# daxiongpro/EPNet

Measured on AMD Instinct MI355X. Metric: SA-stack points/sec per GPU (16384-pt KITTI scene) + % HBM roofline, higher is better.
Workload: dtype f32; 1 GPU; 256 x 16384-pt kitti scenes per GPU per step through the 4-level SA op stack (4 samplings [FPS + centre gather; levels 2-4 nested in level 1 where tie-free] + 8 ball_query + 8 fused groupings [xyz - centre ; features]), pyramid 16384>4096>1024>256>64, radii [[.1,.5],[.5,1],[1,2],[2,4]], nsample [16,32], C=0/96/256/512, HIP-graph launch; levels=4, scenes_per_gpu=256, software_pipelined=True, pipeline_stages=2, parallelism=scene-parallel x1

## Files before the change

epnet_amd/csrc/fps.hip:

```cpp
#include <math.h>

#include <type_traits>

#include "common.h"
#include "dpp.h"
#include "spatial.h"

extern "C" __device__ int epnet_llvm_writelane_i32(int, int, int) __asm("llvm.amdgcn.writelane.i32");

namespace epnet {

__device__ __forceinline__ int writelane_i32(int value, int lane, int old) {
    return epnet_llvm_writelane_i32(value, lane, old);
}

__device__ __forceinline__ unsigned bitrev_lg(unsigned v, int lg) {
    return lg == 0 ? 0u : (__brev(v) >> (32 - lg));
}

__device__ __forceinline__ int wave_max_i32(int v) {
    const int r = row16_max(v);
    const int a = __builtin_amdgcn_readlane(r, 0), b = __builtin_amdgcn_readlane(r, 16);
    const int c = __builtin_amdgcn_readlane(r, 32), d = __builtin_amdgcn_readlane(r, 48);
    return max(max(a, b), max(c, d));
}

constexpr int kIdxBuf = 4096;

__device__ __forceinline__ int fps_point_of(int q, int slot, int R, int J, int lg_bs) {
    const int r = q * R + slot / J;
    return (int)bitrev_lg((unsigned)r, lg_bs) + (slot % J) * (1 << lg_bs);
}

template <int PPT>
__device__ __forceinline__ void find_slot(const int (&t)[PPT], const float (&x)[PPT], const float (&y)[PPT],
                                          const float (&z)[PPT], const int (&g)[(PPT + 3) / 4], int wl, int target,
                                          int &slot, float &sx, float &sy, float &sz) {
    slot = 0;
    sx = sy = sz = 0.f;
    if constexpr (PPT >= 8) {
        constexpr int NG = PPT / 4;
        int grp = 0;
#pragma unroll
        for (int gi = NG - 1; gi >= 0; --gi)
            if (__builtin_amdgcn_readlane(g[gi], wl) == target) grp = gi;
#pragma unroll
        for (int gi = 0; gi < NG; ++gi)
            if (grp == gi) {
#pragma unroll
                for (int j = 4 * gi + 3; j >= 4 * gi; --j)
                    if (__builtin_amdgcn_readlane(t[j], wl) == target) slot = j;
            }
#pragma unroll
        for (int j = 0; j < PPT; ++j)
            if (slot == j) {
                sx = __int_as_float(__builtin_amdgcn_readlane(__float_as_int(x[j]), wl));
                sy = __int_as_float(__builtin_amdgcn_readlane(__float_as_int(y[j]), wl));
                sz = __int_as_float(__builtin_amdgcn_readlane(__float_as_int(z[j]), wl));
            }
    } else {
#pragma unroll
        for (int j = PPT - 1; j >= 0; --j)
            if (__builtin_amdgcn_readlane(t[j], wl) == target) {
                slot = j;
                sx = __int_as_float(__builtin_amdgcn_readlane(__float_as_int(x[j]), wl));
                sy = __int_as_float(__builtin_amdgcn_readlane(__float_as_int(y[j]), wl));
                sz = __int_as_float(__builtin_amdgcn_readlane(__float_as_int(z[j]), wl));
            }
    }
}

__device__ __forceinline__ bool fps_prologue(int m, const int *__restrict__ skip, int *__restrict__ idx_scene,
                                             int *__restrict__ prefix_out, int init) {
    const int have = skip ? skip[blockIdx.x] : 0;
    if (init >= 0) {
        if (threadIdx.x == 0 && prefix_out) prefix_out[blockIdx.x] = have >= m ? have : init;
        for (int i = threadIdx.x; i < min(have, m); i += blockDim.x) idx_scene[i] = i;
    }
    return have >= m;
}

template <int W, int PPT>
__global__ __launch_bounds__(64 * W) void fps_wave_kernel(int n, int m, int lg_bs, const float *__restrict__ xyz,
                                                          float *__restrict__ temp, int *__restrict__ idxs,
                                                          const int *__restrict__ skip, int *__restrict__ prefix_out = nullptr,
                                                          int prologue_init = -1) {
    if (fps_prologue(m, skip, idxs + (size_t)blockIdx.x * m, prefix_out, prologue_init)) return;
    __shared__ int s_val[2][16];
    __shared__ float4 s_rec[2][16];
    __shared__ int s_idx[kIdxBuf];
    constexpr int T = 64 * W;
    const int q = threadIdx.x;
    const int lane = q & 63, wave = q >> 6;
    const int bs = 1 << lg_bs;
    const int R = bs / T, J = (n + bs - 1) / bs;
    const int used = R * J;
    xyz += (size_t)blockIdx.x * n * 3;
    if (temp) temp += (size_t)blockIdx.x * n;
    idxs += (size_t)blockIdx.x * m;
    const int kNeg1 = __float_as_int(-1.f);

    float x[PPT], y[PPT], z[PPT];
    int t[PPT];
#pragma unroll
    for (int s = 0; s < PPT; ++s) {
        const int k = s < used ? fps_point_of(q, s, R, J, lg_bs) : n;
        if (k < n) {
            x[s] = xyz[k * 3 + 0];
            y[s] = xyz[k * 3 + 1];
            z[s] = xyz[k * 3 + 2];
            t[s] = __float_as_int(temp ? temp[k] : 1e10f);
        } else {
            x[s] = y[s] = z[s] = 0.f;
            t[s] = kNeg1;
        }
    }
    if (W > 1 && q < 32) s_val[q >> 4][q & 15] = kNeg1;
    if (q == 0) s_idx[0] = 0;
    float x1 = xyz[0], y1 = xyz[1], z1 = xyz[2];
    __syncthreads();

    for (int it = 1; it < m; ++it) {
        int g[(PPT + 3) / 4];
        int best = kNeg1;
        if constexpr (PPT >= 8) {
#pragma unroll
            for (int gi = 0; gi < PPT / 4; ++gi) {
                int gm = kNeg1;
#pragma unroll
                for (int j = 4 * gi; j < 4 * gi + 4; ++j) {
                    const float dx = x[j] - x1, dy = y[j] - y1, dz = z[j] - z1;
                    const float d = dx * dx + dy * dy + dz * dz;
                    t[j] = min(__float_as_int(d), t[j]);
                    gm = max(gm, t[j]);
                }
                g[gi] = gm;
                best = max(best, gm);
            }
        } else {
#pragma unroll
            for (int j = 0; j < PPT; ++j) {
                const float dx = x[j] - x1, dy = y[j] - y1, dz = z[j] - z1;
                const float d = dx * dx + dy * dy + dz * dz;
                t[j] = min(__float_as_int(d), t[j]);
                best = max(best, t[j]);
            }
            g[0] = best;
        }
        const int wbest = wave_max_i32(best);
        const unsigned long long tied = __ballot(best == wbest);
        const int wl = (int)__builtin_ctzll(tied);
        int slot;
        float sx, sy, sz;
        find_slot<PPT>(t, x, y, z, g, wl, wbest, slot, sx, sy, sz);
        const int code = ((wave * 64 + wl) << 8) | slot;
        if constexpr (W == 1) {
            x1 = sx;
            y1 = sy;
            z1 = sz;
            s_idx[it & (kIdxBuf - 1)] = code;
        } else {
            const int buf = it & 1;
            if (lane == 0) {
                s_val[buf][wave] = wbest;
                s_rec[buf][wave] = make_float4(sx, sy, sz, __int_as_float(code));
            }
            __syncthreads();
            const int wv = s_val[buf][lane & 15];
            const float4 rec = s_rec[buf][lane & 15];
            const int bm = row16_max(wv);
            const unsigned long long wtied = __ballot(wv == bm) & 0xFFFFull;
            const int ww = (int)__builtin_ctzll(wtied);
            x1 = __int_as_float(__builtin_amdgcn_readlane(__float_as_int(rec.x), ww));
            y1 = __int_as_float(__builtin_amdgcn_readlane(__float_as_int(rec.y), ww));
            z1 = __int_as_float(__builtin_amdgcn_readlane(__float_as_int(rec.z), ww));
            const int wcode = __builtin_amdgcn_readlane(__float_as_int(rec.w), ww);
            if (wave == 0) s_idx[it & (kIdxBuf - 1)] = wcode;
        }
        if ((it & (kIdxBuf - 1)) == kIdxBuf - 1 && wave == 0) {
            const int base = it - (kIdxBuf - 1);
            for (int e = lane; e < kIdxBuf; e += 64) {
                const int c = s_idx[e];
                idxs[base + e] = fps_point_of(c >> 8, c & 0xFF, R, J, lg_bs);
            }
        }
    }
    if (wave == 0) {
        const int base = (m - 1) & ~(kIdxBuf - 1);
        for (int e = lane; base + e < m; e += 64) {
            const int c = s_idx[e];
            idxs[base + e] = fps_point_of(c >> 8, c & 0xFF, R, J, lg_bs);
        }
    }
    if (temp) {
#pragma unroll
        for (int s = 0; s < PPT; ++s) {
            const int k = s < used ? fps_point_of(q, s, R, J, lg_bs) : n;
            if (k < n) temp[k] = __int_as_float(t[s]);
        }
    }
}

namespace pruned {

#ifndef EPNET_FPS_PRIO
#define EPNET_FPS_PRIO 3
#endif

#ifdef EPNET_FPS_STATS
__device__ unsigned long long g_stats[16];
#define EPNET_STAMP(var) const unsigned long long var = __builtin_amdgcn_s_memtime()
#define EPNET_ACC(slot, a, b) st_acc[slot] += (unsigned long long)((b) - (a))
#define EPNET_CNT(slot, v) st_acc[slot] += (unsigned long long)(v)
#define EPNET_STATS_BEGIN unsigned long long st_acc[8] = {0, 0, 0, 0, 0, 0, 0, 0}
#define EPNET_STATS_END if ((threadIdx.x & 63) == 0) for (int s_ = 0; s_ < 8; ++s_) atomicAdd(&g_stats[s_], st_acc[s_])
#else
#define EPNET_STAMP(var)
#define EPNET_ACC(slot, a, b)
#define EPNET_CNT(slot, v)
#define EPNET_STATS_BEGIN
#define EPNET_STATS_END
#endif

__device__ __forceinline__ unsigned rank14(int k) { return (bitrev_lg((unsigned)k & 1023u, 10) << 4) | ((unsigned)k >> 10); }
__device__ __forceinline__ int unrank14(unsigned r) { return (int)(bitrev_lg(r >> 4, 10) + ((r & 15u) << 10)); }

template <int G>
__device__ __forceinline__ int group_max(int v) {
    v = max(v, dpp_i32<0xB1>(v));
    v = max(v, dpp_i32<0x4E>(v));
    v = max(v, dpp_i32<0x141>(v));
    if (G >= 16) v = max(v, dpp_i32<0x140>(v));
    if (G >= 32) {
        const auto a = __builtin_amdgcn_permlane16_swap((unsigned)v, (unsigned)v, false, false);
        v = max((int)a[0], (int)a[1]);
    }
    return v;
}
template <int G>
__device__ __forceinline__ float group_minf(float v) {
    v = fminf(v, __int_as_float(dpp_i32<0xB1>(__float_as_int(v))));
    v = fminf(v, __int_as_float(dpp_i32<0x4E>(__float_as_int(v))));
    v = fminf(v, __int_as_float(dpp_i32<0x141>(__float_as_int(v))));
    if (G >= 16) v = fminf(v, __int_as_float(dpp_i32<0x140>(__float_as_int(v))));
    if (G >= 32) {
        const auto a = __builtin_amdgcn_permlane16_swap(__float_as_uint(v), __float_as_uint(v), false, false);
        v = fminf(__uint_as_float(a[0]), __uint_as_float(a[1]));
    }
    return v;
}
template <int G>
__device__ __forceinline__ float group_maxf(float v) { return -group_minf<G>(-v); }

template <int P>
__device__ __forceinline__ int period_max(int v) {
    if (P > 1) v = max(v, dpp_i32<0xB1>(v));
    if (P > 2) v = max(v, dpp_i32<0x4E>(v));
    if (P > 4) v = max(v, dpp_i32<0x124>(v));
    if (P > 8) v = max(v, dpp_i32<0x128>(v));
    return v;
}
template <int P>
__device__ __forceinline__ unsigned period_min(unsigned v) {
    if (P > 1) v = min(v, dpp_u32<0xB1>(v));
    if (P > 2) v = min(v, dpp_u32<0x4E>(v));
    if (P > 4) v = min(v, dpp_u32<0x124>(v));
    if (P > 8) v = min(v, dpp_u32<0x128>(v));
    return v;
}

template <int PPT>
__device__ __forceinline__ unsigned fold_parts(unsigned long long a) {
    if (PPT <= 32) a |= a >> 32;
    if (PPT <= 16) a |= a >> 16;
    if (PPT <= 8) a |= a >> 8;
    return (unsigned)a & (PPT >= 32 ? 0xFFFFFFFFu : ((1u << PPT) - 1u));
}

constexpr int kIdxBufP = 1024;

template <typename VH>
__device__ __forceinline__ unsigned rank_of(const VH &rk2, int j) {
    return ((unsigned)rk2[j >> 1] >> ((j & 1) << 4)) & 0xFFFFu;
}
template <typename VH>
__device__ __forceinline__ void set_rank(VH &rk2, int j, unsigned r) {
    rk2[j >> 1] = (j & 1) ? (int)(((unsigned)rk2[j >> 1] & 0xFFFFu) | (r << 16)) : (int)r;
}

template <int kW, int PPT, typename VF, typename VI, typename VH>
__device__ __forceinline__ void fps_rounds(int m, const VF &x, const VF &y, const VF &z, VI &t, const VH &rk2,
                                           float cx, float cy, float cz, int *__restrict__ idxs,
                                           int *__restrict__ tie_free = nullptr, int known = 0,
                                           const float *__restrict__ xyz_in_order = nullptr, int detect_upto = 0x7fffffff) {
    __shared__ unsigned long long s_key[3];
    __shared__ float4 s_rec[2][64 * kW];
    __shared__ int s_idx[kIdxBufP];
    const int q = threadIdx.x;
    const int lane = q & 63, wave = q >> 6;
    const int sub = lane & (PPT - 1);
    const int kNeg1 = __float_as_int(-1.f);

    int bm = kNeg1;
    float lox = 0.f, hix = 0.f, loy = 0.f, hiy = 0.f, loz = 0.f, hiz = 0.f;
    for (int j = 0; j < PPT; ++j) {
        const float xj = x[j], yj = y[j], zj = z[j];
        const int tj = t[j];
        const bool real = tj != kNeg1;
        const float mnx = group_minf<PPT>(real ? xj : 3.4e38f), mxx = group_maxf<PPT>(real ? xj : -3.4e38f);
        const float mny = group_minf<PPT>(real ? yj : 3.4e38f), mxy = group_maxf<PPT>(real ? yj : -3.4e38f);
        const float mnz = group_minf<PPT>(real ? zj : 3.4e38f), mxz = group_maxf<PPT>(real ? zj : -3.4e38f);
        const int gm = group_max<PPT>(tj);
        if (sub == j) {
            const bool any = gm != kNeg1;
            bm = gm;
            lox = any ? mnx : 0.f; hix = any ? mxx : 0.f;
            loy = any ? mny : 0.f; hiy = any ? mxy : 0.f;
            loz = any ? mnz : 0.f; hiz = any ? mxz : 0.f;
        }
    }
    if (q < 3) s_key[q] = 0ull;
    if (q == 0) s_idx[0] = 0;
    if (known > kIdxBufP || known > m || !xyz_in_order) known = 0;
    for (int i = q; i < known; i += 64 * kW) s_idx[i] = (int)rank14(i);
    __syncthreads();
    for (int it = 1; it < known; ++it) {
        const float px = __builtin_amdgcn_fmed3f(cx, lox, hix), py = __builtin_amdgcn_fmed3f(cy, loy, hiy),
                    pz = __builtin_amdgcn_fmed3f(cz, loz, hiz);
        const float bdx = px - cx, bdy = py - cy, bdz = pz - cz;
        const float L = bdx * bdx + bdy * bdy + bdz * bdz;
        unsigned active = fold_parts<PPT>(__ballot(__float_as_int(L) < bm));
        const float nx = xyz_in_order[it * 3 + 0], ny = xyz_in_order[it * 3 + 1], nz = xyz_in_order[it * 3 + 2];
        while (active) {
            const int j = (int)__builtin_ctz(active);
            active &= active - 1u;
            const float xj = x[j], yj = y[j], zj = z[j];
            const int told = t[j];
            __builtin_amdgcn_sched_barrier(0);
            const float dx = xj - cx, dy = yj - cy, dz = zj - cz;
            const float d = dx * dx + dy * dy + dz * dz;
            const int tj = min(__float_as_int(d), told);
            t[j] = tj;
            const int gm = group_max<PPT>(tj);
            bm = (sub == j) ? gm : bm;
// ... 388 lines not shown
                const int e1 = two ? s_ * 64 + (int)__builtin_ctzll(act) : e0;
                act &= act - 1ull;
                const Row r0 = load_row(e0);
                Row r1 = r0;
                if (two) r1 = load_row(e1);
                finish(e0, r0, true, cx, cy, cz);
                if (two) finish(e1, r1, true, cx, cy, cz);
            }
        }
        if (stale) {
            stale = false;
            int lmax = bm[0];
#pragma unroll
            for (int s_ = 1; s_ < kBPL; ++s_) lmax = max(lmax, bm[s_]);
            wbest = wave_max_all(lmax);
            unsigned lrank = 0xFFFFFFFFu;
            float lx = 0.f, ly = 0.f, lz = 0.f;
#pragma unroll
            for (int s_ = 0; s_ < kBPL; ++s_) {
                const bool take = bm[s_] == wbest && bm[s_] != kNeg1 && brank[s_] < lrank;
                lrank = take ? brank[s_] : lrank;
                lx = take ? bxx[s_] : lx;
                ly = take ? byy[s_] : ly;
                lz = take ? bzz[s_] : lz;
            }
            unsigned long long cand = __ballot(lrank != 0xFFFFFFFFu);
            if (cand & (cand - 1ull)) {
                const unsigned rmin = wave_min_all(lrank);
                cand = __ballot(lrank == rmin);
            }
            publisher = cand != 0ull && lane == (int)__builtin_ctzll(cand);
            pub_rank = lrank;
            pub_x = lx; pub_y = ly; pub_z = lz;
        }
        const int buf = it & 1;
        if (publisher) {
            s_rec[buf][wave] = make_float4(pub_x, pub_y, pub_z, 0.f);
            const unsigned long long key =
                ((unsigned long long)(unsigned)wbest << 32) | (unsigned long long)(((0xFFFFu - pub_rank) << 4) | (unsigned)wave);
            __hip_atomic_fetch_max(&s_key[kb], key, __ATOMIC_RELAXED, __HIP_MEMORY_SCOPE_WORKGROUP);
        }
        __syncthreads();
        const unsigned klo = (unsigned)s_key[kb];
        const float4 rec = s_rec[buf][klo & 15u];
        cx = rec.x;
        cy = rec.y;
        cz = rec.z;
        const int kb2 = kb == 0 ? 2 : kb - 1;
        kb = kb == 2 ? 0 : kb + 1;
        if (wave == 0) {
            s_idx[it & (kIdxBufP - 1)] = (int)(0xFFFFu - (klo >> 4));
            if (lane == 0) s_key[kb2] = 0ull;
            if ((it & (kIdxBufP - 1)) == kIdxBufP - 1) {
                const int base = it - (kIdxBufP - 1);
                for (int e = lane; e < kIdxBufP; e += 64) idxs[base + e] = unrank16((unsigned)s_idx[e]);
            }
        }
    }
    if (wave == 0) {
        const int base = (m - 1) & ~(kIdxBufP - 1);
        for (int e = lane; base + e < m; e += 64) idxs[base + e] = unrank16((unsigned)s_idx[e]);
    }
    __builtin_amdgcn_s_setprio(0);
    for (int e = 0; e < nmine; ++e) {
        const int pos = (bid(e) << 6) + lane;
        if (pos < n) temp[__float_as_int(sorted[pos].w)] = tsort[pos];
    }
}

}


__device__ __forceinline__ unsigned fps_rank(int k, int lg) {
    return (bitrev_lg((unsigned)k & ((1u << lg) - 1u), lg) << 20) | ((unsigned)k >> lg);
}

__device__ __forceinline__ int fps_unrank(unsigned rank, int lg) {
    return (int)(bitrev_lg(rank >> 20, lg) + ((rank & 0xFFFFFu) << lg));
}

__device__ __forceinline__ long long wave_max_i64(long long v) {
#pragma unroll
    for (int off = 32; off >= 1; off >>= 1) {
        const long long o = __shfl_xor(v, off, 64);
        v = o > v ? o : v;
    }
    return v;
}

__global__ __launch_bounds__(1024) void fps_stream_kernel(int n, int m, int lg_bs, const float *__restrict__ xyz,
                                                          float *__restrict__ temp, int *__restrict__ idxs,
                                                          const int *__restrict__ skip) {
    if (skip && skip[blockIdx.x] >= m) return;
    __shared__ long long red[2][16];
    const int BS = blockDim.x;
    const int q = threadIdx.x;
    const int lane = q & 63, wave = q >> 6;
    xyz += (size_t)blockIdx.x * n * 3;
    temp += (size_t)blockIdx.x * n;
    idxs += (size_t)blockIdx.x * m;
    if (q < 32) red[q >> 4][q & 15] = (long long)0x8000000000000000ull;
    if (q == 0) idxs[0] = 0;
    float x1 = xyz[0], y1 = xyz[1], z1 = xyz[2];
    __syncthreads();
    for (int it = 1; it < m; ++it) {
        float best = -1.f;
        int bestk = q;
        for (int k = q; k < n; k += BS) {
            const float dx = xyz[k * 3 + 0] - x1, dy = xyz[k * 3 + 1] - y1, dz = xyz[k * 3 + 2] - z1;
            const float d = dx * dx + dy * dy + dz * dz;
            const float d2 = fminf(d, temp[k]);
            temp[k] = d2;
            bestk = d2 > best ? k : bestk;
            best = d2 > best ? d2 : best;
        }
        const unsigned rank = fps_rank(bestk, lg_bs);
        long long key = ((long long)__float_as_int(best) << 32) | (long long)(0x7FFFFFFFu - rank);
        key = wave_max_i64(key);
        if (lane == 0) red[it & 1][wave] = key;
        __syncthreads();
        long long kk = red[it & 1][lane & 15];
#pragma unroll
        for (int off = 8; off >= 1; off >>= 1) {
            const long long o = __shfl_xor(kk, off, 64);
            kk = o > kk ? o : kk;
        }
        const unsigned wr = 0x7FFFFFFFu - (unsigned)(kk & 0xFFFFFFFFll);
        const int old = __builtin_amdgcn_readfirstlane(fps_unrank(wr, lg_bs));
        x1 = xyz[old * 3 + 0];
        y1 = xyz[old * 3 + 1];
        z1 = xyz[old * 3 + 2];
        if (q == 0) idxs[it] = old;
    }
}

static int ref_block_lg(int work_size) {
    int pow_2 = (int)(std::log(static_cast<double>(work_size)) / std::log(2.0));
    if (pow_2 > 10) pow_2 = 10;
    if (pow_2 < 0) pow_2 = 0;
    return pow_2;
}

}

using namespace epnet;

__global__ void fps_prefix_kernel(int m, const int *__restrict__ skip, int *__restrict__ idx, int *__restrict__ prefix_out, int init);

static bool fps_prune_applies(int n, int m) {
    return tuning(kFpsPrune) != 0 && n > 1024 && n > tuning(kFpsPruneMin) && n <= 16384 && m > 1;
}

static int fps_plain(int b, int n, int m, const float *xyz, float *temp, int *idx, const int *skip, int *prefix_out,
                     epnet_stream_t stream, int prefix_cap = 0x7fffffff, int prologue_init = -1) {
    EPNET_REQUIRE(b >= 0 && n >= 1 && m >= 0);
    if (b == 0 || m == 0) return EPNET_OK;
    EPNET_REQUIRE(xyz && idx);
    if ((long long)n > (1ll << 20) * 1024) return EPNET_ELIMIT;
    hipStream_t s = (hipStream_t)stream;
    const int lg = ref_block_lg(n);
    const int bs_ref = 1 << lg;
    dim3 grid(b);
    const int J = div_up(n, bs_ref);
    auto prefix_first = [&]() -> int {
        if (prologue_init < 0) return EPNET_OK;
        hipLaunchKernelGGL(fps_prefix_kernel, dim3(b), dim3(256), 0, s, m, skip, idx, prefix_out, prologue_init);
        return check_launch("sampling prefix");
    };
    if (fps_prune_applies(n, m)) {
        if (int rc = prefix_first()) return rc;
        int waves = n > 8192 ? 8 : 4;
        const int w = tuning(kFpsPwaves);
        if (w > 0 && div_up(n, 64 * w) <= 32) waves = w;
        const int ppt_need = div_up(n, 64 * waves);
        const int ppt = ppt_need <= 8 ? 8 : ppt_need <= 16 ? 16 : 32;
        const size_t lds = (size_t)(kCells + kCells / (kCells / (64 * waves)) + 64) * sizeof(int) + (size_t)64 * waves * ppt * 2;
#define EPNET_FPS_PRUNED(W_, P_) \
    hipLaunchKernelGGL((pruned::fps_pruned_kernel<W_, P_>), grid, dim3(64 * W_), lds, s, n, m, xyz, temp, idx, skip, prefix_out, prefix_cap)
        if (waves == 8) {
            if (ppt == 8) EPNET_FPS_PRUNED(8, 8);
            else if (ppt == 16) EPNET_FPS_PRUNED(8, 16);
            else EPNET_FPS_PRUNED(8, 32);
        } else {
            if (ppt == 8) EPNET_FPS_PRUNED(4, 8);
            else if (ppt == 16) EPNET_FPS_PRUNED(4, 16);
            else EPNET_FPS_PRUNED(4, 32);
        }
#undef EPNET_FPS_PRUNED
        return check_launch("furthest_point_sampling");
    }
    if (bs_ref >= 64 && J <= 16) {
        int waves = bs_ref / 64;
        for (int w = 1; w <= bs_ref / 64; w *= 2)
            if ((bs_ref / (64 * w)) * J <= 16) {
                waves = w;
                break;
            }
        if (n > 512 && b <= 512 && bs_ref / 64 >= 8 && waves < 8) waves = 8;
        const int w = tuning(kFpsWaves);
        if (w >= 1 && w <= bs_ref / 64 && (bs_ref / (64 * w)) * J <= 16) waves = w;
        const int ppt = (bs_ref / (64 * waves)) * J;
#define EPNET_FPS_LAUNCH(W_, P_) \
    hipLaunchKernelGGL((fps_wave_kernel<W_, P_>), grid, dim3(64 * W_), 0, s, n, m, lg, xyz, temp, idx, skip, prefix_out, prologue_init)
#define EPNET_FPS_PPT(W_)                      \
    do {                                       \
        if (ppt <= 1) EPNET_FPS_LAUNCH(W_, 1); \
        else if (ppt <= 2) EPNET_FPS_LAUNCH(W_, 2); \
        else if (ppt <= 4) EPNET_FPS_LAUNCH(W_, 4); \
        else if (ppt <= 8) EPNET_FPS_LAUNCH(W_, 8); \
        else EPNET_FPS_LAUNCH(W_, 16);         \
    } while (0)
        switch (waves) {
            case 1: EPNET_FPS_PPT(1); break;
            case 2: EPNET_FPS_PPT(2); break;
            case 4: EPNET_FPS_PPT(4); break;
            case 8: EPNET_FPS_PPT(8); break;
            default: EPNET_FPS_PPT(16); break;
        }
#undef EPNET_FPS_PPT
#undef EPNET_FPS_LAUNCH
        return check_launch("furthest_point_sampling");
    }
    float *tbuf = temp;
    if (!tbuf) return EPNET_EINVAL;
    if (int rc = prefix_first()) return rc;
    const int bs = bs_ref < 64 ? 64 : bs_ref;
    hipLaunchKernelGGL(fps_stream_kernel, grid, dim3(bs), 0, s, n, m, lg, xyz, tbuf, idx, skip);
    return check_launch("furthest_point_sampling");
}

extern "C" int epnet_furthest_point_sampling(int b, int n, int m, const float *xyz, float *temp, int *idx,
                                             epnet_stream_t stream) {
    return fps_plain(b, n, m, xyz, temp, idx, nullptr, nullptr, stream, 0x7fffffff);
}

static bool fps_detects_ties(int n, int m, bool indexed) {
    if (indexed) return m > 1 && n > 1024 && n <= 16384;
    return fps_prune_applies(n, m);
}

__global__ __launch_bounds__(256) void fps_prefix_kernel(int m, const int *__restrict__ skip, int *__restrict__ idx,
                                                         int *__restrict__ prefix_out, int init) {
    const int bs = blockIdx.x;
    const int have = skip ? skip[bs] : 0;
    const bool known = have >= m;
    if (threadIdx.x == 0 && prefix_out) prefix_out[bs] = known ? have : init;
    for (int i = threadIdx.x; i < min(have, m); i += 256) idx[(size_t)bs * m + i] = i;
}

__global__ __launch_bounds__(256) void gather_centres_kernel(int n, int m, const float *__restrict__ xyz,
                                                             const int *__restrict__ idx, float *__restrict__ out) {
    const int bs = blockIdx.y;
    const int e = blockIdx.x * 256 + threadIdx.x;
    if (e >= m * 3) return;
    const int i = e / 3, a = e - i * 3;
    out[(size_t)bs * m * 3 + e] = xyz[((size_t)bs * n + idx[(size_t)bs * m + i]) * 3 + a];
}

__global__ __launch_bounds__(256) void gather_centres4_kernel(int n, int m, const float *__restrict__ xyz,
                                                              const int *__restrict__ idx, float *__restrict__ out) {
    const int bs = blockIdx.y;
    const int i4 = blockIdx.x * 256 + threadIdx.x;
    if (i4 * 4 >= m) return;
    const int4 ids = reinterpret_cast<const int4 *>(idx + (size_t)bs * m)[i4];
    const float *src = xyz + (size_t)bs * n * 3;
    const float *p0 = src + (size_t)ids.x * 3, *p1 = src + (size_t)ids.y * 3, *p2 = src + (size_t)ids.z * 3, *p3 = src + (size_t)ids.w * 3;
    const float a0 = p0[0], a1 = p0[1], a2 = p0[2], b0 = p1[0], b1 = p1[1], b2 = p1[2];
    const float c0 = p2[0], c1 = p2[1], c2 = p2[2], d0 = p3[0], d1 = p3[1], d2 = p3[2];
    float4 *dst = reinterpret_cast<float4 *>(out + ((size_t)bs * m + (size_t)i4 * 4) * 3);
    dst[0] = make_float4(a0, a1, a2, b0);
    dst[1] = make_float4(b1, b2, c0, c1);
    dst[2] = make_float4(c2, d0, d1, d2);
}

static void launch_gather_centres(int b, int n, int m, const float *xyz, const int *idx, float *new_xyz, hipStream_t s) {
    if ((m & 3) == 0 && (((uintptr_t)idx | (uintptr_t)new_xyz) & 15) == 0)
        hipLaunchKernelGGL(gather_centres4_kernel, dim3(div_up(m / 4, 256), b), dim3(256), 0, s, n, m, xyz, idx, new_xyz);
    else
        hipLaunchKernelGGL(gather_centres_kernel, dim3(div_up(m * 3, 256), b), dim3(256), 0, s, n, m, xyz, idx, new_xyz);
}

static int fps_over_index(int b, int n, int m, const float *xyz, void *index, size_t index_bytes, float *temp, int *idx,
                          float *new_xyz, hipStream_t s, const int *skip = nullptr, int *prefix_out = nullptr,
                          int prefix_cap = 0x7fffffff) {
    const size_t need = scene_index_bytes(b, n);
    int rc;
    const bool plain = need == 0 || !index || n <= 1024 || m <= 1 || (n > 16384 && !temp);
    int fold_init = -1;
    if (skip || prefix_out) {
        EPNET_REQUIRE(idx && b <= 65535);
        if (prefix_cap < 1) prefix_cap = 0x7fffffff;
        fold_init = fps_detects_ties(n, m, !plain) ? m : 0;
    }
    if (fold_init >= 0 && m == 0) {
        hipLaunchKernelGGL(fps_prefix_kernel, dim3(b), dim3(256), 0, s, m, skip, idx, prefix_out, fold_init);
        return check_launch("sampling prefix");
    }
    if (plain) {
        rc = fps_plain(b, n, m, xyz, temp, idx, skip, prefix_out, (epnet_stream_t)s, prefix_cap, fold_init);
    } else {
        EPNET_REQUIRE(idx);
        if (index_bytes < need) return EPNET_ENOMEM;
        const float4 *sorted = (const float4 *)index;
        dim3 grid(b);
        if (n > 16384) {
            EPNET_REQUIRE(xyz);
            if (fold_init >= 0) {
                hipLaunchKernelGGL(fps_prefix_kernel, dim3(b), dim3(256), 0, s, m, skip, idx, prefix_out, fold_init);
                rc = check_launch("sampling prefix");
                if (rc) return rc;
            }
            const int np = scene_index_np(n);
            const float *bucket_boxes = (const float *)(sorted + (size_t)b * np);
            float *tsort = scene_index_sampling_scratch(b, n, index);
            hipLaunchKernelGGL(pruned::fps_bigscene_kernel<16>, grid, dim3(1024), 0, s, n, np, m, xyz, sorted, bucket_boxes, temp, tsort, idx, skip);
        } else {
#define EPNET_FPS_INDEXED(W_, P_)                                                                                                     \
    hipLaunchKernelGGL((pruned::fps_indexed_kernel<W_, P_>), grid, dim3(64 * W_), 0, s, n, m, sorted, temp, idx, skip, prefix_out, xyz, \
                       prefix_cap, fold_init)
            switch (scene_index_np(n)) {
                case 2048: EPNET_FPS_INDEXED(4, 8); break;
                case 4096: EPNET_FPS_INDEXED(4, 16); break;
                case 8192: EPNET_FPS_INDEXED(4, 32); break;
                default: EPNET_FPS_INDEXED(8, 32); break;
            }
#undef EPNET_FPS_INDEXED
        }
        rc = check_launch("furthest_point_sampling");
    }
    if (rc || !new_xyz) return rc;
    if (m == 0) return EPNET_OK;
    EPNET_REQUIRE(xyz && b <= 65535);
    launch_gather_centres(b, n, m, xyz, idx, new_xyz, s);
    return check_launch("sample_centres gather");
}

extern "C" int epnet_furthest_point_sampling_indexed(int b, int n, int m, const float *xyz, void *index,
                                                     size_t index_bytes, float *temp, int *idx,
                                                     epnet_stream_t stream) {
    return fps_over_index(b, n, m, xyz, index, index_bytes, temp, idx, nullptr, (hipStream_t)stream);
}

extern "C" int epnet_sample_centres(int b, int n, int m, const float *xyz, void *index, size_t index_bytes,
                                    float *temp, int *idx, float *new_xyz, epnet_stream_t stream) {
    EPNET_REQUIRE(b >= 0 && n >= 1 && m >= 0);
    if (b == 0 || m == 0) return EPNET_OK;
    EPNET_REQUIRE(xyz && idx && new_xyz);
    return fps_over_index(b, n, m, xyz, index, index_bytes, temp, idx, new_xyz, (hipStream_t)stream);
}

extern "C" int epnet_sample_centres_chain(int b, int n, int m, const float *xyz, void *index, size_t index_bytes,
                                          float *temp, int *idx, float *new_xyz, const int *prefix_in, int *prefix_out,
                                          int prefix_cap, epnet_stream_t stream) {
    EPNET_REQUIRE(b >= 0 && n >= 1 && m >= 0);
    if (b == 0 || m == 0) return EPNET_OK;
    EPNET_REQUIRE(xyz && idx);
    if (m > n) prefix_in = nullptr;
    return fps_over_index(b, n, m, xyz, index, index_bytes, temp, idx, new_xyz, (hipStream_t)stream, prefix_in, prefix_out,
                          prefix_cap);
}
```

epnet_amd/csrc/group.hip:

```cpp

#include "common.h"
#include "spatial.h"
#include "runsum.h"

namespace epnet {

constexpr int kGThreads = 256;
constexpr int kGChan = 16;

__global__ __launch_bounds__(kGThreads) void gather_rows_vec4_kernel(int c, int n, int p, size_t ostride,
                                                                     const float *__restrict__ points,
                                                                     const int *__restrict__ idx,
                                                                     float *__restrict__ out) {
    int wg_x, wg_y, bs;
    xcd_scene_map3(wg_x, wg_y, bs);
    const int c0 = wg_y * kGChan;
    const int q4 = wg_x * kGThreads + threadIdx.x;
    if (q4 * 4 >= p) return;
    const int4 id = *reinterpret_cast<const int4 *>(idx + (size_t)bs * p + (size_t)q4 * 4);
    const int cend = min(c, c0 + kGChan);
    const float *src = points + ((size_t)bs * c + c0) * n;
    float *dst = out + (size_t)bs * ostride + (size_t)c0 * p + (size_t)q4 * 4;
#pragma unroll 4
    for (int ci = c0; ci < cend; ++ci) {
        float4 v;
        v.x = src[id.x];
        v.y = src[id.y];
        v.z = src[id.z];
        v.w = src[id.w];
        *reinterpret_cast<float4 *>(dst) = v;
        src += n;
        dst += p;
    }
}

__global__ __launch_bounds__(kGThreads) void gather_rows_scalar_kernel(int c, int n, int p, size_t ostride,
                                                                       const float *__restrict__ points,
                                                                       const int *__restrict__ idx,
                                                                       float *__restrict__ out) {
    int wg_x, wg_y, bs;
    xcd_scene_map3(wg_x, wg_y, bs);
    const int c0 = wg_y * kGChan;
    const int q = wg_x * kGThreads + threadIdx.x;
    if (q >= p) return;
    const int id = idx[(size_t)bs * p + q];
    const int cend = min(c, c0 + kGChan);
    for (int ci = c0; ci < cend; ++ci)
        out[(size_t)bs * ostride + (size_t)ci * p + q] = points[((size_t)bs * c + ci) * n + id];
}

#ifndef EPNET_GATHER_STAGE_UNROLL
#define EPNET_STAGE_PRAGMA
#else
#define EPNET_STAGE_STR2(x) #x
#define EPNET_STAGE_STR(x) EPNET_STAGE_STR2(unroll x)
#define EPNET_STAGE_PRAGMA _Pragma(EPNET_STAGE_STR(EPNET_GATHER_STAGE_UNROLL))
#endif
#ifndef EPNET_GATHER_LDS_BUDGET_KB
#define EPNET_GATHER_LDS_BUDGET_KB 64
#endif
#ifndef EPNET_GATHER_LDS_THREADS
#define EPNET_GATHER_LDS_THREADS 256
#endif
#ifndef EPNET_GATHER_LDS_UNROLL
#define EPNET_GATHER_LDS_UNROLL 1
#endif
constexpr int kGLdsThreads = EPNET_GATHER_LDS_THREADS;
__device__ __forceinline__ void stage_quads(const float *__restrict__ src, int groups, int n, float4 *__restrict__ s_quad,
                                            int threads) {
    const int n4 = n >> 2;
    for (int e = threadIdx.x; e < groups * n4; e += threads) {
        const int g = e / n4, j4 = e - g * n4;
        const float4 *row = reinterpret_cast<const float4 *>(src + (size_t)g * 4 * n) + j4;
        const float4 a = row[0], b4 = row[n4], cc = row[2 * n4], d = row[3 * n4];
        float4 *dst = s_quad + (size_t)g * n + j4 * 4;
        dst[0] = make_float4(a.x, b4.x, cc.x, d.x);
        dst[1] = make_float4(a.y, b4.y, cc.y, d.y);
        dst[2] = make_float4(a.z, b4.z, cc.z, d.z);
        dst[3] = make_float4(a.w, b4.w, cc.w, d.w);
    }
}

__device__ __forceinline__ void serve_quads(const float4 *__restrict__ quad, int groups, int n, int4 id, float *__restrict__ dst,
                                            int p) {
#pragma unroll 1
    for (int g = 0; g < groups; ++g) {
        const float4 v0 = quad[id.x], v1 = quad[id.y], v2 = quad[id.z], v3 = quad[id.w];
        store_stream(dst, v0.x, v1.x, v2.x, v3.x);
        store_stream(dst + p, v0.y, v1.y, v2.y, v3.y);
        store_stream(dst + 2 * (size_t)p, v0.z, v1.z, v2.z, v3.z);
        store_stream(dst + 3 * (size_t)p, v0.w, v1.w, v2.w, v3.w);
        quad += n;
        dst += 4 * (size_t)p;
    }
}

template <bool QUAD>
__global__ __launch_bounds__(kGLdsThreads) void gather_rows_lds_kernel(int c, int n, int p, int rows, int tile, size_t ostride,
                                                                    const float *__restrict__ points,
                                                                    const int *__restrict__ idx,
                                                                    float *__restrict__ out) {
    extern __shared__ float s_rows[];
    int wg_x, wg_y, bs;
    xcd_scene_map3(wg_x, wg_y, bs);
    const int c0 = wg_y * rows;
    const int nr = min(rows, c - c0);
    const float *src = points + ((size_t)bs * c + c0) * n;
    const int total = nr * n;
    if (QUAD) {
        stage_quads(src, nr >> 2, n, reinterpret_cast<float4 *>(s_rows), kGLdsThreads);
    } else if ((n & 3) == 0 && ((uintptr_t)src & 15) == 0) {
        const float4 *src4 = reinterpret_cast<const float4 *>(src);
        float4 *dst4 = reinterpret_cast<float4 *>(s_rows);
        EPNET_STAGE_PRAGMA
        for (int e = threadIdx.x; e < total / 4; e += kGLdsThreads) dst4[e] = src4[e];
    } else {
        for (int e = threadIdx.x; e < total; e += kGLdsThreads) s_rows[e] = src[e];
    }
    __syncthreads();
    const int q_begin = wg_x * tile, q_end = min(p, q_begin + tile);
    const int *ix = idx + (size_t)bs * p;
    float *dst_base = out + (size_t)bs * ostride + (size_t)c0 * p;
    for (int q = q_begin + threadIdx.x * 4; q < q_end; q += kGLdsThreads * 4) {
        const int4 id = *reinterpret_cast<const int4 *>(ix + q);
        float *dst = dst_base + q;
        if (QUAD) {
            serve_quads(reinterpret_cast<const float4 *>(s_rows), nr >> 2, n, id, dst, p);
            continue;
        }
        const float *row = s_rows;
#pragma unroll EPNET_GATHER_LDS_UNROLL
        for (int r = 0; r < nr; ++r) {
            float4 v;
            v.x = row[id.x];
            v.y = row[id.y];
            v.z = row[id.z];
            v.w = row[id.w];
            store_stream(dst, v.x, v.y, v.z, v.w);
            row += n;
            dst += p;
        }
    }
}

#ifndef EPNET_GATHER_LDS2_UNROLL
#define EPNET_GATHER_LDS2_UNROLL 1
#endif
constexpr long long kGatherLds2MinPositions = 3 * kGLdsThreads * 4;
template <bool QUAD>
__global__ __launch_bounds__(kGLdsThreads) void gather_rows_lds2_kernel(int c, int n, int rows, const float *__restrict__ points,
                                                                        int p0, size_t ostride0, const int *__restrict__ idx0,
                                                                        float *__restrict__ out0, int p1, size_t ostride1,
                                                                        const int *__restrict__ idx1, float *__restrict__ out1) {
    extern __shared__ float s_rows[];
    int wg_x, bs;
    xcd_scene_map(wg_x, bs);
    const int c0 = wg_x * rows;
    const int nr = min(rows, c - c0);
    const float *src = points + ((size_t)bs * c + c0) * n;
    const int total = nr * n;
    if (QUAD) {
        stage_quads(src, nr >> 2, n, reinterpret_cast<float4 *>(s_rows), kGLdsThreads);
    } else if ((n & 3) == 0 && ((uintptr_t)src & 15) == 0) {
        const float4 *src4 = reinterpret_cast<const float4 *>(src);
        float4 *dst4 = reinterpret_cast<float4 *>(s_rows);
        EPNET_STAGE_PRAGMA
        for (int e = threadIdx.x; e < total / 4; e += kGLdsThreads) dst4[e] = src4[e];
    } else {
        for (int e = threadIdx.x; e < total; e += kGLdsThreads) s_rows[e] = src[e];
    }
    __syncthreads();
#pragma unroll 1
    for (int set = 0; set < 2; ++set) {
        const int p = set ? p1 : p0;
        const int *ix = (set ? idx1 : idx0) + (size_t)bs * p;
        float *dst_base = (set ? out1 : out0) + (size_t)bs * (set ? ostride1 : ostride0) + (size_t)c0 * p;
        for (int q = threadIdx.x * 4; q < p; q += kGLdsThreads * 4) {
            const int4 id = *reinterpret_cast<const int4 *>(ix + q);
            float *dst = dst_base + q;
            if (QUAD) {
                serve_quads(reinterpret_cast<const float4 *>(s_rows), nr >> 2, n, id, dst, p);
                continue;
            }
            const float *row = s_rows;
#pragma unroll EPNET_GATHER_LDS2_UNROLL
            for (int r = 0; r < nr; ++r) {
                float4 v;
                v.x = row[id.x];
                v.y = row[id.y];
                v.z = row[id.z];
                v.w = row[id.w];
                store_stream(dst, v.x, v.y, v.z, v.w);
                row += n;
                dst += p;
            }
        }
    }
}

__global__ __launch_bounds__(kGThreads) void scatter_rows_lds_kernel(int c, int n, int p, int rows, size_t gstride,
                                                                     const float *__restrict__ grad_out,
                                                                     const int *__restrict__ idx,
                                                                     float *__restrict__ grad_points) {
    extern __shared__ float acc[];
    const int bs = blockIdx.y;
    const int c0 = blockIdx.x * rows;
    const int nr = min(rows, c - c0);
    for (int e = threadIdx.x; e < nr * n; e += kGThreads) acc[e] = 0.f;
    __syncthreads();
    const int *ix = idx + (size_t)bs * p;
    const float *go = grad_out + (size_t)bs * gstride + (size_t)c0 * p;
    for (int q = threadIdx.x; q < p; q += kGThreads) {
        const int id = ix[q];
        for (int r = 0; r < nr; ++r) atomicAdd(&acc[r * n + id], go[(size_t)r * p + q]);
    }
    __syncthreads();
    float *gp = grad_points + ((size_t)bs * c + c0) * n;
    for (int e = threadIdx.x; e < nr * n; e += kGThreads) gp[e] += acc[e];
}

__global__ __launch_bounds__(kGThreads) void scatter_rows_atomic_kernel(int c, int n, int p, size_t gstride,
                                                                        const float *__restrict__ grad_out,
                                                                        const int *__restrict__ idx,
                                                                        float *__restrict__ grad_points) {
    const int bs = blockIdx.z, ci = blockIdx.y;
    const int q = blockIdx.x * kGThreads + threadIdx.x;
    if (q >= p) return;
    atomicAdd(grad_points + ((size_t)bs * c + ci) * n + idx[(size_t)bs * p + q],
              grad_out[(size_t)bs * gstride + (size_t)ci * p + q]);
}

__global__ __launch_bounds__(kGThreads) void group_xyz_centred_kernel(int n, int npoints, int nsample, size_t ostride,
                                                                      const float *__restrict__ xyz,
                                                                      const float *__restrict__ new_xyz,
                                                                      const int *__restrict__ idx, float *__restrict__ out) {
    int wg_x, bs;
    xcd_scene_map(wg_x, bs);
    const int p = npoints * nsample;
    const int q = wg_x * kGThreads + threadIdx.x;
    if (q >= p) return;
    const int id = idx[(size_t)bs * p + q];
    const int ci = q / nsample;
    const float *pt = xyz + ((size_t)bs * n + id) * 3;
    const float *ce = new_xyz + ((size_t)bs * npoints + ci) * 3;
    float *dst = out + (size_t)bs * ostride + q;
    dst[0] = pt[0] - ce[0];
    dst[(size_t)p] = pt[1] - ce[1];
    dst[(size_t)p * 2] = pt[2] - ce[2];
}

__global__ __launch_bounds__(kGThreads) void group_xyz_centred_vec4_kernel(int n, int npoints, int nsample, size_t ostride,
                                                                           const float *__restrict__ xyz,
                                                                           const float *__restrict__ new_xyz,
                                                                           const int *__restrict__ idx,
                                                                           float *__restrict__ out) {
    int wg_x, bs;
    xcd_scene_map(wg_x, bs);
    const int p = npoints * nsample;
    const int q = (wg_x * kGThreads + threadIdx.x) * 4;
    if (q >= p) return;
    const int4 id = *reinterpret_cast<const int4 *>(idx + (size_t)bs * p + q);
    const float *base = xyz + (size_t)bs * n * 3;
    const float *ce = new_xyz + ((size_t)bs * npoints + q / nsample) * 3;
    const float cx = ce[0], cy = ce[1], cz = ce[2];
    const float *p0 = base + (size_t)id.x * 3, *p1 = base + (size_t)id.y * 3, *p2 = base + (size_t)id.z * 3,
                *p3 = base + (size_t)id.w * 3;
    float *dst = out + (size_t)bs * ostride + q;
    *reinterpret_cast<float4 *>(dst) = make_float4(p0[0] - cx, p1[0] - cx, p2[0] - cx, p3[0] - cx);
    *reinterpret_cast<float4 *>(dst + (size_t)p) = make_float4(p0[1] - cy, p1[1] - cy, p2[1] - cy, p3[1] - cy);
    *reinterpret_cast<float4 *>(dst + (size_t)p * 2) = make_float4(p0[2] - cz, p1[2] - cz, p2[2] - cz, p3[2] - cz);
}

__global__ __launch_bounds__(kGLdsThreads) void group_linear_lds_kernel(int c, int n, int npoints, int nsample, int rows, int tile,
                                                                        const float *__restrict__ z, const float *__restrict__ xyz,
                                                                        const float *__restrict__ new_xyz, const int *__restrict__ idx,
                                                                        const float *__restrict__ wx, const float *__restrict__ bias,
                                                                        float *__restrict__ out) {
    extern __shared__ float s_rows[];
    const int bs = blockIdx.z;
    const int c0 = blockIdx.y * rows;
    const int nr = min(rows, c - c0);
    const int p = npoints * nsample;
    const float *src = z + ((size_t)bs * c + c0) * n;
    const int total = nr * n;
    if ((n & 3) == 0 && ((uintptr_t)src & 15) == 0) {
        const float4 *src4 = reinterpret_cast<const float4 *>(src);
        float4 *dst4 = reinterpret_cast<float4 *>(s_rows);
        EPNET_STAGE_PRAGMA
        for (int e = threadIdx.x; e < total / 4; e += kGLdsThreads) dst4[e] = src4[e];
    } else {
        for (int e = threadIdx.x; e < total; e += kGLdsThreads) s_rows[e] = src[e];
    }
    __syncthreads();
    const int q_begin = blockIdx.x * tile, q_end = min(p, q_begin + tile);
    const int *ix = idx + (size_t)bs * p;
    const float *pts = xyz + (size_t)bs * n * 3;
    float *dst_base = out + ((size_t)bs * c + c0) * p;
    for (int q = q_begin + threadIdx.x * 4; q < q_end; q += kGLdsThreads * 4) {
        const int4 id = *reinterpret_cast<const int4 *>(ix + q);
        const float *ce = new_xyz + ((size_t)bs * npoints + q / nsample) * 3;
        const float cx = ce[0], cy = ce[1], cz = ce[2];
        const float *p0 = pts + (size_t)id.x * 3, *p1 = pts + (size_t)id.y * 3, *p2 = pts + (size_t)id.z * 3, *p3 = pts + (size_t)id.w * 3;
        const float dx0 = p0[0] - cx, dy0 = p0[1] - cy, dz0 = p0[2] - cz;
        const float dx1 = p1[0] - cx, dy1 = p1[1] - cy, dz1 = p1[2] - cz;
        const float dx2 = p2[0] - cx, dy2 = p2[1] - cy, dz2 = p2[2] - cz;
        const float dx3 = p3[0] - cx, dy3 = p3[1] - cy, dz3 = p3[2] - cz;
        float *dst = dst_base + q;
        const float *row = s_rows;
#pragma unroll 2
        for (int r = 0; r < nr; ++r) {
            const float w0 = wx[(c0 + r) * 3], w1 = wx[(c0 + r) * 3 + 1], w2 = wx[(c0 + r) * 3 + 2];
            float4 v;
            v.x = row[id.x] + (w0 * dx0 + w1 * dy0 + w2 * dz0);
            v.y = row[id.y] + (w0 * dx1 + w1 * dy1 + w2 * dz1);
            v.z = row[id.z] + (w0 * dx2 + w1 * dy2 + w2 * dz2);
            v.w = row[id.w] + (w0 * dx3 + w1 * dy3 + w2 * dz3);
            if (bias) {
                const float bv = bias[c0 + r];
                v.x += bv; v.y += bv; v.z += bv; v.w += bv;
            }
            store_stream(dst, v.x, v.y, v.z, v.w);
            row += n;
            dst += p;
        }
    }
}

__global__ __launch_bounds__(kGThreads) void group_linear_scalar_kernel(int c, int n, int npoints, int nsample,
                                                                        const float *__restrict__ z, const float *__restrict__ xyz,
                                                                        const float *__restrict__ new_xyz, const int *__restrict__ idx,
                                                                        const float *__restrict__ wx, const float *__restrict__ bias,
                                                                        float *__restrict__ out) {
    const int bs = blockIdx.z;
    const int c0 = blockIdx.y * kGChan;
    const int p = npoints * nsample;
    const int q = blockIdx.x * kGThreads + threadIdx.x;
    if (q >= p) return;
    const int id = idx[(size_t)bs * p + q];
    const float *pt = xyz + ((size_t)bs * n + id) * 3;
    const float *ce = new_xyz + ((size_t)bs * npoints + q / nsample) * 3;
    const float dx = pt[0] - ce[0], dy = pt[1] - ce[1], dz = pt[2] - ce[2];
    const int cend = min(c, c0 + kGChan);
    for (int ci = c0; ci < cend; ++ci) {
        float v = z[((size_t)bs * c + ci) * n + id] + (wx[ci * 3] * dx + wx[ci * 3 + 1] * dy + wx[ci * 3 + 2] * dz);
        if (bias) v += bias[ci];
        out[((size_t)bs * c + ci) * p + q] = v;
    }
}

constexpr int kGwRows = 8;
// ... 476 lines not shown
```

Before: 1.442 billion points/s.

## Fuse centre gather into wave FPS and software-pipeline LDS gather index loads

The wave FPS kernel now writes the selected centre coordinates directly when a new_xyz buffer is given, so the separate centre-gather launch is skipped on that path. The LDS grouping gather kernels are restructured to prefetch index vectors one or more iterations ahead, to precompute byte offsets, and to fully unroll the row-group loop for common channel counts (4, 16 and 32 rows). The aim is to cut one kernel launch plus a re-read of indices, and to hide index-load latency behind the LDS reads and streaming stores. The cost is extra template instantiations, higher register pressure, and scattered global reads of xyz inside the FPS tail.

New measurement: 1.469 billion points/s, median of 6. 1.02x the previous value.

```diff
diff --git a/epnet_amd/csrc/fps.hip b/epnet_amd/csrc/fps.hip
--- a/epnet_amd/csrc/fps.hip
+++ b/epnet_amd/csrc/fps.hip
@@ -84,8 +84,15 @@
 __global__ __launch_bounds__(64 * W) void fps_wave_kernel(int n, int m, int lg_bs, const float *__restrict__ xyz,
                                                           float *__restrict__ temp, int *__restrict__ idxs,
                                                           const int *__restrict__ skip, int *__restrict__ prefix_out = nullptr,
-                                                          int prologue_init = -1) {
-    if (fps_prologue(m, skip, idxs + (size_t)blockIdx.x * m, prefix_out, prologue_init)) return;
+                                                          int prologue_init = -1, float *__restrict__ new_xyz = nullptr) {
+    if (new_xyz) new_xyz += (size_t)blockIdx.x * m * 3;
+    if (fps_prologue(m, skip, idxs + (size_t)blockIdx.x * m, prefix_out, prologue_init)) {
+        if (new_xyz) {
+            const float *src = xyz + (size_t)blockIdx.x * n * 3;
+            for (int e = threadIdx.x; e < m * 3; e += blockDim.x) new_xyz[e] = src[e];
+        }
+        return;
+    }
     __shared__ int s_val[2][16];
     __shared__ float4 s_rec[2][16];
     __shared__ int s_idx[kIdxBuf];
@@ -181,7 +188,14 @@
             const int base = it - (kIdxBuf - 1);
             for (int e = lane; e < kIdxBuf; e += 64) {
                 const int c = s_idx[e];
-                idxs[base + e] = fps_point_of(c >> 8, c & 0xFF, R, J, lg_bs);
+                const int k = fps_point_of(c >> 8, c & 0xFF, R, J, lg_bs);
+                idxs[base + e] = k;
+                if (new_xyz) {
+                    float *dst = new_xyz + (size_t)(base + e) * 3;
+                    dst[0] = xyz[k * 3 + 0];
+                    dst[1] = xyz[k * 3 + 1];
+                    dst[2] = xyz[k * 3 + 2];
+                }
             }
         }
     }
@@ -189,7 +203,14 @@
         const int base = (m - 1) & ~(kIdxBuf - 1);
         for (int e = lane; base + e < m; e += 64) {
             const int c = s_idx[e];
-            idxs[base + e] = fps_point_of(c >> 8, c & 0xFF, R, J, lg_bs);
+            const int k = fps_point_of(c >> 8, c & 0xFF, R, J, lg_bs);
+            idxs[base + e] = k;
+            if (new_xyz) {
+                float *dst = new_xyz + (size_t)(base + e) * 3;
+                dst[0] = xyz[k * 3 + 0];
+                dst[1] = xyz[k * 3 + 1];
+                dst[2] = xyz[k * 3 + 2];
+            }
         }
     }
     if (temp) {
@@ -884,7 +905,9 @@
 }
 
 static int fps_plain(int b, int n, int m, const float *xyz, float *temp, int *idx, const int *skip, int *prefix_out,
-                     epnet_stream_t stream, int prefix_cap = 0x7fffffff, int prologue_init = -1) {
+                     epnet_stream_t stream, int prefix_cap = 0x7fffffff, int prologue_init = -1, float *new_xyz = nullptr,
+                     bool *wrote_centres = nullptr) {
+    if (wrote_centres) *wrote_centres = false;
     EPNET_REQUIRE(b >= 0 && n >= 1 && m >= 0);
     if (b == 0 || m == 0) return EPNET_OK;
     EPNET_REQUIRE(xyz && idx);
@@ -933,7 +956,8 @@
         if (w >= 1 && w <= bs_ref / 64 && (bs_ref / (64 * w)) * J <= 16) waves = w;
         const int ppt = (bs_ref / (64 * waves)) * J;
 #define EPNET_FPS_LAUNCH(W_, P_) \
-    hipLaunchKernelGGL((fps_wave_kernel<W_, P_>), grid, dim3(64 * W_), 0, s, n, m, lg, xyz, temp, idx, skip, prefix_out, prologue_init)
+    hipLaunchKernelGGL((fps_wave_kernel<W_, P_>), grid, dim3(64 * W_), 0, s, n, m, lg, xyz, temp, idx, skip, prefix_out, prologue_init, \
+                       new_xyz)
 #define EPNET_FPS_PPT(W_)                      \
     do {                                       \
         if (ppt <= 1) EPNET_FPS_LAUNCH(W_, 1); \
@@ -951,6 +975,7 @@
         }
 #undef EPNET_FPS_PPT
 #undef EPNET_FPS_LAUNCH
+        if (wrote_centres) *wrote_centres = new_xyz != nullptr;
         return check_launch("furthest_point_sampling");
     }
     float *tbuf = temp;
@@ -1019,6 +1044,7 @@
     int rc;
     const bool plain = need == 0 || !index || n <= 1024 || m <= 1 || (n > 16384 && !temp);
     int fold_init = -1;
+    bool wrote_centres = false;
     if (skip || prefix_out) {
         EPNET_REQUIRE(idx && b <= 65535);
         if (prefix_cap < 1) prefix_cap = 0x7fffffff;
@@ -1029,7 +1055,7 @@
         return check_launch("sampling prefix");
     }
     if (plain) {
-        rc = fps_plain(b, n, m, xyz, temp, idx, skip, prefix_out, (epnet_stream_t)s, prefix_cap, fold_init);
+        rc = fps_plain(b, n, m, xyz, temp, idx, skip, prefix_out, (epnet_stream_t)s, prefix_cap, fold_init, new_xyz, &wrote_centres);
     } else {
         EPNET_REQUIRE(idx);
         if (index_bytes < need) return EPNET_ENOMEM;
@@ -1060,7 +1086,7 @@
         }
         rc = check_launch("furthest_point_sampling");
     }
-    if (rc || !new_xyz) return rc;
+    if (rc || !new_xyz || wrote_centres) return rc;
     if (m == 0) return EPNET_OK;
     EPNET_REQUIRE(xyz && b <= 65535);
     launch_gather_centres(b, n, m, xyz, idx, new_xyz, s);
diff --git a/epnet_amd/csrc/group.hip b/epnet_amd/csrc/group.hip
--- a/epnet_amd/csrc/group.hip
+++ b/epnet_amd/csrc/group.hip
@@ -1,3 +1,5 @@
+
+#include <type_traits>
 
 #include "common.h"
 #include "spatial.h"
@@ -65,6 +67,9 @@
 #ifndef EPNET_GATHER_LDS_UNROLL
 #define EPNET_GATHER_LDS_UNROLL 1
 #endif
+#ifndef EPNET_GATHER_ONE_GROUP_PASSES
+#define EPNET_GATHER_ONE_GROUP_PASSES 2
+#endif
 constexpr int kGLdsThreads = EPNET_GATHER_LDS_THREADS;
 __device__ __forceinline__ void stage_quads(const float *__restrict__ src, int groups, int n, float4 *__restrict__ s_quad,
                                             int threads) {
@@ -81,18 +86,108 @@
     }
 }
 
-__device__ __forceinline__ void serve_quads(const float4 *__restrict__ quad, int groups, int n, int4 id, float *__restrict__ dst,
-                                            int p) {
+__device__ __forceinline__ void serve_quad_group(const char *__restrict__ quad, int4 o, float *__restrict__ dst, int p) {
+    const float4 v0 = *reinterpret_cast<const float4 *>(quad + o.x), v1 = *reinterpret_cast<const float4 *>(quad + o.y),
+                 v2 = *reinterpret_cast<const float4 *>(quad + o.z), v3 = *reinterpret_cast<const float4 *>(quad + o.w);
+    store_stream(dst, v0.x, v1.x, v2.x, v3.x);
+    store_stream(dst + p, v0.y, v1.y, v2.y, v3.y);
+    store_stream(dst + 2 * (size_t)p, v0.z, v1.z, v2.z, v3.z);
+    store_stream(dst + 3 * (size_t)p, v0.w, v1.w, v2.w, v3.w);
+}
+
+template <bool QUAD, int G>
+__device__ __forceinline__ void serve_vector(const float *__restrict__ s_rows, int nr, int n, int4 o, float *__restrict__ dst,
+                                             int p) {
+    const char *row = reinterpret_cast<const char *>(s_rows);
+    if (QUAD) {
+        if (G > 0) {
+#pragma unroll
+            for (int g = 0; g < G; ++g) {
+                serve_quad_group(row, o, dst, p);
+                row += (size_t)n * 16;
+                dst += 4 * (size_t)p;
+                __builtin_amdgcn_sched_barrier(0);
+            }
+        } else {
 #pragma unroll 1
-    for (int g = 0; g < groups; ++g) {
-        const float4 v0 = quad[id.x], v1 = quad[id.y], v2 = quad[id.z], v3 = quad[id.w];
-        store_stream(dst, v0.x, v1.x, v2.x, v3.x);
-        store_stream(dst + p, v0.y, v1.y, v2.y, v3.y);
-        store_stream(dst + 2 * (size_t)p, v0.z, v1.z, v2.z, v3.z);
-        store_stream(dst + 3 * (size_t)p, v0.w, v1.w, v2.w, v3.w);
-        quad += n;
-        dst += 4 * (size_t)p;
-    }
+            for (int g = 0; g < (nr >> 2); ++g) {
+                serve_quad_group(row, o, dst, p);
+                row += (size_t)n * 16;
+                dst += 4 * (size_t)p;
+            }
+        }
+        return;
+    }
+#pragma unroll EPNET_GATHER_LDS_UNROLL
+    for (int r = 0; r < nr; ++r) {
+        float4 v;
+        v.x = *reinterpret_cast<const float *>(row + o.x);
+        v.y = *reinterpret_cast<const float *>(row + o.y);
+        v.z = *reinterpret_cast<const float *>(row + o.z);
+        v.w = *reinterpret_cast<const float *>(row + o.w);
+        store_stream(dst, v.x, v.y, v.z, v.w);
+        row += (size_t)n * 4;
+        dst += p;
+    }
+}
+
+__device__ __forceinline__ int4 load_ids(const int *__restrict__ ix, int q, int ahead, int q_last) {
+    return *reinterpret_cast<const int4 *>(ix + (min(q, q_last - ahead) + ahead));
+}
+
+template <bool QUAD>
+__device__ __forceinline__ int4 lds_offsets(int4 id) {
+    constexpr int kShift = QUAD ? 4 : 2;
+    int4 o = make_int4(id.x << kShift, id.y << kShift, id.z << kShift, id.w << kShift);
+    asm volatile("" : "+v"(o.x), "+v"(o.y), "+v"(o.z), "+v"(o.w));
+    return o;
+}
+
+template <bool QUAD, int G, int U>
+__device__ __forceinline__ void serve_span(const float *__restrict__ s_rows, int nr, int n, const int *__restrict__ ix,
+                                           int q_begin, int q_end, float *__restrict__ dst_base, int p) {
+    constexpr int kStep = kGLdsThreads * 4;
+    const int q_last = q_end - 4;
+    int q = q_begin + threadIdx.x * 4;
+    int4 o[U];
+#pragma unroll
+    for (int u = 0; u < U; ++u) o[u] = load_ids(ix, q, u * kStep, q_last);
+#pragma unroll
+    for (int u = 0; u < U; ++u) o[u] = lds_offsets<QUAD>(o[u]);
+    if (U > 1) {
+#pragma unroll 1
+        for (int k = (q_end - q_begin) / (U * kStep); k > 0; --k) {
+            int4 nx[U];
+#pragma unroll
+            for (int u = 0; u < U; ++u) nx[u] = load_ids(ix, q, (U + u) * kStep, q_last);
+#pragma unroll
+            for (int u = 0; u < U; ++u) serve_vector<QUAD, G>(s_rows, nr, n, o[u], dst_base + q + u * kStep, p);
+#pragma unroll
+            for (int u = 0; u < U; ++u) o[u] = lds_offsets<QUAD>(nx[u]);
+            q += U * kStep;
+        }
+    }
+    int4 cur = o[0];
+#pragma unroll 1
+    for (; q < q_end; q += kStep) {
+        const int4 nx = load_ids(ix, q, kStep, q_last);
+        serve_vector<QUAD, G>(s_rows, nr, n, cur, dst_base + q, p);
+        cur = lds_offsets<QUAD>(nx);
+    }
+}
+
+template <int V>
+using gather_const = std::integral_constant<int, V>;
+template <bool QUAD, typename Serve>
+__device__ __forceinline__ void for_row_groups(int nr, Serve serve) {
+    if (QUAD && nr == 4)
+        serve(gather_const<1>(), gather_const<EPNET_GATHER_ONE_GROUP_PASSES>());
+    else if (QUAD && nr == 16)
+        serve(gather_const<4>(), gather_const<1>());
+    else if (QUAD && nr == 32)
+        serve(gather_const<8>(), gather_const<1>());
+    else
+        serve(gather_const<0>(), gather_const<1>());
 }
 
 template <bool QUAD>
@@ -121,31 +216,12 @@
     const int q_begin = wg_x * tile, q_end = min(p, q_begin + tile);
     const int *ix = idx + (size_t)bs * p;
     float *dst_base = out + (size_t)bs * ostride + (size_t)c0 * p;
-    for (int q = q_begin + threadIdx.x * 4; q < q_end; q += kGLdsThreads * 4) {
-        const int4 id = *reinterpret_cast<const int4 *>(ix + q);
-        float *dst = dst_base + q;
-        if (QUAD) {
-            serve_quads(reinterpret_cast<const float4 *>(s_rows), nr >> 2, n, id, dst, p);
-            continue;
-        }
-        const float *row = s_rows;
-#pragma unroll EPNET_GATHER_LDS_UNROLL
-        for (int r = 0; r < nr; ++r) {
-            float4 v;
-            v.x = row[id.x];
-            v.y = row[id.y];
-            v.z = row[id.z];
-            v.w = row[id.w];
-            store_stream(dst, v.x, v.y, v.z, v.w);
-            row += n;
-            dst += p;
-        }
-    }
-}
-
-#ifndef EPNET_GATHER_LDS2_UNROLL
-#define EPNET_GATHER_LDS2_UNROLL 1
-#endif
+    if (q_begin >= q_end) return;
+    for_row_groups<QUAD>(nr, [&](auto g, auto u) {
+        serve_span<QUAD, decltype(g)::value, decltype(u)::value>(s_rows, nr, n, ix, q_begin, q_end, dst_base, p);
+    });
+}
+
 constexpr long long kGatherLds2MinPositions = 3 * kGLdsThreads * 4;
 template <bool QUAD>
 __global__ __launch_bounds__(kGLdsThreads) void gather_rows_lds2_kernel(int c, int n, int rows, const float *__restrict__ points,
@@ -170,32 +246,15 @@
         for (int e = threadIdx.x; e < total; e += kGLdsThreads) s_rows[e] = src[e];
     }
     __syncthreads();
+    for_row_groups<QUAD>(nr, [&](auto g, auto u) {
 #pragma unroll 1
-    for (int set = 0; set < 2; ++set) {
-        const int p = set ? p1 : p0;
-        const int *ix = (set ? idx1 : idx0) + (size_t)bs * p;
-        float *dst_base = (set ? out1 : out0) + (size_t)bs * (set ? ostride1 : ostride0) + (size_t)c0 * p;
-        for (int q = threadIdx.x * 4; q < p; q += kGLdsThreads * 4) {
-            const int4 id = *reinterpret_cast<const int4 *>(ix + q);
-            float *dst = dst_base + q;
-            if (QUAD) {
-                serve_quads(reinterpret_cast<const float4 *>(s_rows), nr >> 2, n, id, dst, p);
-                continue;
-            }
-            const float *row = s_rows;
-#pragma unroll EPNET_GATHER_LDS2_UNROLL
-            for (int r = 0; r < nr; ++r) {
-                float4 v;
-                v.x = row[id.x];
-                v.y = row[id.y];
-                v.z = row[id.z];
-                v.w = row[id.w];
-                store_stream(dst, v.x, v.y, v.z, v.w);
-                row += n;
-                dst += p;
-            }
-        }
-    }
+        for (int set = 0; set < 2; ++set) {
+            const int p = set ? p1 : p0;
+            const int *ix = (set ? idx1 : idx0) + (size_t)bs * p;
+            float *dst_base = (set ? out1 : out0) + (size_t)bs * (set ? ostride1 : ostride0) + (size_t)c0 * p;
+            if (p > 0) serve_span<QUAD, decltype(g)::value, decltype(u)::value>(s_rows, nr, n, ix, 0, p, dst_base, p);
+        }
+    });
 }
 
 __global__ __launch_bounds__(kGThreads) void scatter_rows_lds_kernel(int c, int n, int p, int rows, size_t gstride,
```
